# SuperScientificSoftwareLaboratory/PanguLU

Hardware: AMD Instinct MI355X
Metric: numeric factorisation GFLOP/s (pangulu_gstrf, R64) (higher is better)
Workload: dtype f64

## Files before the change

pangulu_amd/csrc/platform/pg_hip_front.h:

```cpp
#pragma once

#define FR_TILE 128
#define FR_KS 16
#define FR_LDA 144
#define FR_STAGE_DOUBLES (FR_KS * FR_LDA + FR_TILE * FR_KS)
#define FR_THREADS 512

typedef const char __attribute__((address_space(1))) *fr_gptr;
typedef void __attribute__((address_space(3))) *fr_lptr;

#ifndef FR_ISSUE_FIRST
#define FR_ISSUE_FIRST 0
#endif
#define FR_ORDER (FR_ISSUE_FIRST ? 0 : 1)
#ifndef FR_PRELOAD
#define FR_PRELOAD 1
#endif

template <int STAGES, bool PREFETCH, int ORDER>
__device__ __forceinline__ void fr_front_item(double *lds, const SsssmTaskD *__restrict__ tasks, int nb, const SsssmWorkD &G,
                                              unsigned long long *__restrict__ product_counter)
{
    const int tiles = nb / FR_TILE;
    const int tile = (int)G.tile;
    const int tid = threadIdx.x, lane = tid & 63;
    const int wave = __builtin_amdgcn_readfirstlane(tid >> 6);
    const int M0 = (tile % tiles) * FR_TILE, N0 = (tile / tiles) * FR_TILE;
    const int wm = (wave & 1) * 64, wn = (wave >> 1) * 32;
    const int l15 = lane & 15, l4 = lane >> 4;
    const int ntask = (int)(G.task_end - G.task_begin);
    const int steps_shift = nb == 256 ? 4 : 3;
    const int steps_per_task = 1 << steps_shift;
    const int T = ntask << steps_shift;
    const SsssmTaskD *my_tasks = tasks + G.task_begin;

    const unsigned a_voff = (unsigned)lane * 16u;
    const int bc = lane >> 3, bj = lane & 7;
    unsigned b_voff[2];
#pragma unroll
    for (int par = 0; par < 2; par++)
        b_voff[par] = ((unsigned)bc * (unsigned)nb + 2u * (unsigned)(bj ^ ((4 * par + (bc >> 1)) & 7))) * 8u;

    auto issue = [&](int st, fr_gptr pa, fr_gptr pb)
    {
        const int k0 = (st & (steps_per_task - 1)) * FR_KS;
        double *stage = lds + (st % STAGES) * FR_STAGE_DOUBLES;
#pragma unroll
        for (int h = 0; h < 2; h++)
        {
            const int k = wave + 8 * h;
            const fr_gptr src = dg_scalar_base(pa + ((size_t)(k0 + k) * nb + M0) * 8) + a_voff;
            __builtin_amdgcn_global_load_lds((const void __attribute__((address_space(1))) *)src, (fr_lptr)(stage + k * FR_LDA), 16, 0, 0);
        }
#pragma unroll
        for (int h = 0; h < 2; h++)
        {
            const int g = wave + 8 * h;
            const fr_gptr src = dg_scalar_base(pb + ((size_t)(N0 + 8 * g) * nb + k0) * 8) + b_voff[wave & 1];
            __builtin_amdgcn_global_load_lds((const void __attribute__((address_space(1))) *)src, (fr_lptr)(stage + FR_KS * FR_LDA + g * 128), 16, 0, 0);
        }
    };

    double __attribute__((address_space(1))) *C = (double __attribute__((address_space(1))) *)reinterpret_cast<double *>(G.cdense);
    const unsigned c_voff = ((unsigned)l4 * (unsigned)nb + (unsigned)l15) * 8u;
#define FR_C(ni_, mi_, r_)                                                                           \
    (*(double __attribute__((address_space(1))) *)(dg_scalar_base((const char __attribute__((address_space(1))) *)C +                    \
                                                                  ((size_t)(N0 + wn + (ni_) * 16 + 4 * (r_)) * nb + M0 + wm) * 8) + \
                                                   dg_lane_offset(c_voff) + (mi_) * 128))
    const bool preload = FR_PRELOAD && !G.atomic && T > 0;
    v4f64 acc[2][4];
#pragma unroll
    for (int ni = 0; ni < 2; ni++)
#pragma unroll
        for (int mi = 0; mi < 4; mi++)
        {
            if (preload)
            {
#pragma unroll
                for (int r = 0; r < 4; r++)
                    acc[ni][mi][r] = FR_C(ni, mi, r);
            }
            else
                acc[ni][mi] = (v4f64){0.0, 0.0, 0.0, 0.0};
        }

    fr_gptr pa_rq = nullptr, pb_rq = nullptr;
    if (T > 0)
    {
        pa_rq = (fr_gptr)reinterpret_cast<const char *>(my_tasks[0].a.val);
        pb_rq = (fr_gptr)reinterpret_cast<const char *>(my_tasks[0].b.val);
    }
#if PG_PLANES > 1
    bool add = T > 0 && my_tasks[0].sign < 0;
#endif

#pragma unroll
    for (int p = 0; p < STAGES - 1; p++)
        if (p < T)
            issue(p, pa_rq, pb_rq);

    const int a_frag = l4 * FR_LDA + wm + l15;
    int b_frag[2][2];
#pragma unroll
    for (int ni = 0; ni < 2; ni++)
    {
        const int n = wn + ni * 16 + l15;
        b_frag[ni][0] = FR_KS * FR_LDA + n * 16 + (l4 & 1);
        b_frag[ni][1] = (n >> 1) & 7;
    }

    for (int st = 0; st < T; st++)
    {
        const int rq = st + STAGES - 1;
        fr_gptr pa_nx = pa_rq, pb_nx = pb_rq;
        if (((rq + 1) & (steps_per_task - 1)) == 0 && rq + 1 < T)
        {
            const SsssmTaskD &Tn = my_tasks[(rq + 1) >> steps_shift];
            pa_nx = (fr_gptr)reinterpret_cast<const char *>(Tn.a.val);
            pb_nx = (fr_gptr)reinterpret_cast<const char *>(Tn.b.val);
        }
#if PG_PLANES > 1
        bool add_nx = add;
        if (((st + 1) & (steps_per_task - 1)) == 0 && st + 1 < T)
            add_nx = my_tasks[(st + 1) >> steps_shift].sign < 0;
#endif
        const int ahead = min(STAGES - 2, T - 1 - st);
        if (STAGES >= 4 && ahead >= 2)
            asm volatile("s_waitcnt vmcnt(8)" ::: "memory");
        else if (STAGES >= 3 && ahead >= 1)
            asm volatile("s_waitcnt vmcnt(4)" ::: "memory");
        else
            asm volatile("s_waitcnt vmcnt(0)" ::: "memory");
        __builtin_amdgcn_s_barrier();
        const bool request = rq < T;
        if (ORDER == 0 && request)
            issue(rq, pa_rq, pb_rq);
        const double *sA = lds + (st % STAGES) * FR_STAGE_DOUBLES;
#if PG_PLANES > 1
#define FR_MFMA(ni_, mi_, fb_, fa_)                                                                                        \
    if (add)                                                                                                                \
        acc[ni_][mi_] = __builtin_amdgcn_mfma_f64_16x16x4f64(fb_, fa_, acc[ni_][mi_], 0, 0, 0);                          \
    else                                                                                                                    \
        acc[ni_][mi_] = __builtin_amdgcn_mfma_f64_16x16x4f64(fb_, fa_, acc[ni_][mi_], 0, 0, DG_NEG_A);
#else
#define FR_MFMA(ni_, mi_, fb_, fa_) acc[ni_][mi_] = __builtin_amdgcn_mfma_f64_16x16x4f64(fb_, fa_, acc[ni_][mi_], 0, 0, DG_NEG_A);
#endif
#define FR_READ(fa_, fb_, kq_)                                                                        \
    {                                                                                                 \
        _Pragma("unroll") for (int mi = 0; mi < 4; mi++)(fa_)[mi] = sA[a_frag + (kq_) * 4 * FR_LDA + mi * 16]; \
        _Pragma("unroll") for (int ni = 0; ni < 2; ni++)(fb_)[ni] = sA[b_frag[ni][0] + 2 * ((2 * (kq_) + (l4 >> 1)) ^ b_frag[ni][1])]; \
    }
#define FR_REQUEST_BEHIND(kq_)                   \
    if (ORDER == 1 && (kq_) == 0 && request)     \
        issue(rq, pa_rq, pb_rq);
        if (PREFETCH)
        {
            double fa[2][4], fb[2][2];
            FR_READ(fa[0], fb[0], 0)
#pragma unroll
            for (int kq = 0; kq < FR_KS / 4; kq++)
            {
                if (kq + 1 < FR_KS / 4)
                    FR_READ(fa[(kq + 1) & 1], fb[(kq + 1) & 1], kq + 1)
#pragma unroll
                for (int ni = 0; ni < 2; ni++)
#pragma unroll
                    for (int mi = 0; mi < 4; mi++)
                    {
                        FR_MFMA(ni, mi, fb[kq & 1][ni], fa[kq & 1][mi])
                    }
                FR_REQUEST_BEHIND(kq)
            }
        }
        else
        {
#pragma unroll
            for (int kq = 0; kq < FR_KS / 4; kq++)
            {
                double fa[4], fb[2];
                FR_READ(fa, fb, kq)
#pragma unroll
                for (int ni = 0; ni < 2; ni++)
#pragma unroll
                    for (int mi = 0; mi < 4; mi++)
                    {
                        FR_MFMA(ni, mi, fb[ni], fa[mi])
                    }
                FR_REQUEST_BEHIND(kq)
            }
        }
#undef FR_REQUEST_BEHIND
#undef FR_READ
#undef FR_MFMA
        pa_rq = pa_nx;
        pb_rq = pb_nx;
#if PG_PLANES > 1
        add = add_nx;
#endif
    }
    if (product_counter && lane == 0 && T)
        atomicAdd(product_counter, (unsigned long long)(8 * T));

    if (preload)
    {
#pragma unroll
        for (int ni = 0; ni < 2; ni++)
#pragma unroll
            for (int mi = 0; mi < 4; mi++)
#pragma unroll
                for (int r = 0; r < 4; r++)
                    FR_C(ni, mi, r) = acc[ni][mi][r];
        return;
    }
#pragma unroll
    for (int ni = 0; ni < 2; ni++)
    {
        if (G.atomic)
        {
#pragma unroll
            for (int mi = 0; mi < 4; mi++)
#pragma unroll
                for (int r = 0; r < 4; r++)
                    atomicAdd((double *)&FR_C(ni, mi, r), acc[ni][mi][r]);
            continue;
        }
        double old[4][4];
#pragma unroll
        for (int mi = 0; mi < 4; mi++)
#pragma unroll
            for (int r = 0; r < 4; r++)
                old[mi][r] = FR_C(ni, mi, r);
#pragma unroll
        for (int mi = 0; mi < 4; mi++)
#pragma unroll
            for (int r = 0; r < 4; r++)
                FR_C(ni, mi, r) = old[mi][r] + acc[ni][mi][r];
    }
#undef FR_C
}

template <int STAGES, bool PREFETCH>
__global__ __launch_bounds__(FR_THREADS, (STAGES <= 2 ? 4 : 2)) void ssssm_front_f64_kernel(const SsssmTaskD *__restrict__ tasks, int nb, const SsssmWorkD *__restrict__ work,
                                                                     unsigned long long *__restrict__ product_counter, unsigned unit)
{
    __shared__ __align__(16) double lds[STAGES * FR_STAGE_DOUBLES];
    const int tiles = nb / FR_TILE;
    const unsigned bid = logical_block_id(unit ? unit : (unsigned)(tiles * tiles));
    const SsssmWorkD G = work[bid];
    fr_front_item<STAGES, PREFETCH, FR_ORDER>(lds, tasks, nb, G, product_counter);
}

#define TL_WINDOW 16
#ifndef TL_MARK
#define TL_PROBE_DECL
#define TL_MARK(i)
#define TL_PROBE_STEP
#define TL_PROBE_FLUSH
#endif
#ifndef TL_ITEM
#define TL_ITEM_DECL
#define TL_ITEM(i)
#define TL_ITEM_COUNT
#endif
#define TV_STEPS (TL_WINDOW * 16)
__global__ __launch_bounds__(FR_THREADS, 4) void ssssm_tilesv_f64_kernel(const SsssmTaskD *__restrict__ tasks, int nb, const SsssmWorkD *__restrict__ work,
                                                                          unsigned long long *__restrict__ product_counter, unsigned unit)
{
    __shared__ __align__(16) double lds[2 * FR_STAGE_DOUBLES];
    __shared__ unsigned long long s_spa[TV_STEPS], s_spb[TV_STEPS];
    __shared__ u32 s_step[TV_STEPS];
    __shared__ u32 s_cnt[FR_THREADS / 64];
#if PG_PLANES > 1
    __shared__ double s_sign[TL_WINDOW];
#endif
    const int tiles = nb / FR_TILE;
    const unsigned bid = logical_block_id(unit ? unit : (unsigned)(tiles * tiles));
    const SsssmWorkD G = work[bid];
    const int tile = (int)G.tile;
    const int tid = threadIdx.x, lane = tid & 63;
    const int wave = __builtin_amdgcn_readfirstlane(tid >> 6);
    const int M0 = (tile % tiles) * FR_TILE, N0 = (tile / tiles) * FR_TILE;
    const int wr = wave & 1, wc = wave >> 1;
    const int l15 = lane & 15, l4 = lane >> 4;
    if (G.pad_ != 0)
    {
        fr_front_item<2, true, FR_ORDER>(lds, tasks, nb, G, product_counter);
        return;
    }
    const int ntask = (int)(G.task_end - G.task_begin);
    const int nslab = nb / FR_KS;
    const SsssmTaskD *my_tasks = tasks + G.task_begin;

    const unsigned a_voff = (unsigned)lane * 16u;
    const int a_piece = lane >> 3;
    const int bc = lane >> 3, bj = lane & 7;
    const unsigned b_voff = ((unsigned)bc * (unsigned)nb + 2u * (unsigned)(bj ^ ((4 * (wave & 1) + (bc >> 1)) & 7))) * 8u;

    v4f64 acc[2][4];
#pragma unroll
    for (int ni = 0; ni < 2; ni++)
#pragma unroll
        for (int mi = 0; mi < 4; mi++)
            acc[ni][mi] = (v4f64){0.0, 0.0, 0.0, 0.0};
    unsigned touched = 0, nprod = 0;

    const int a_frag = l4 * FR_LDA + wr * 16 + l15;
    int b_frag[2][2];
#pragma unroll
    for (int ni = 0; ni < 2; ni++)
    {
        const int n = (wc + 4 * ni) * 16 + l15;
        b_frag[ni][0] = FR_KS * FR_LDA + n * 16 + (l4 & 1);
        b_frag[ni][1] = (n >> 1) & 7;
    }

    auto uniform64 = [&](unsigned long long v) -> fr_gptr
    { return (fr_gptr)(((unsigned long long)(unsigned)__builtin_amdgcn_readfirstlane((int)(v >> 32)) << 32) | (unsigned)__builtin_amdgcn_readfirstlane((int)v)); };
    auto issue = [&](unsigned w, fr_gptr pa, fr_gptr pb, int stage_no)
    {
        const unsigned ab = w & 0xFFu, bb = (w >> 8) & 0xFFu;
        const int k0 = (int)((w >> 16) & 15u) * FR_KS;
        double *stage = lds + stage_no * FR_STAGE_DOUBLES;
        const bool a_live = (ab >> a_piece) & 1u;
#pragma unroll
        for (int h = 0; h < 2; h++)
        {
            const int k = wave + 8 * h;
            const unsigned off = a_live ? (unsigned)(((k0 + k) * nb + M0) * 8) + a_voff : 0u;
            __builtin_amdgcn_global_load_lds((const void __attribute__((address_space(1))) *)(dg_scalar_base(pa) + off), (fr_lptr)(stage + k * FR_LDA), 16, 0, 0);
        }
#pragma unroll
        for (int h = 0; h < 2; h++)
        {
            const int g = wave + 8 * h;
            if (!((bb >> (g >> 1)) & 1u))
                continue;
            const unsigned off = (unsigned)(((N0 + 8 * g) * nb + k0) * 8) + b_voff;
            __builtin_amdgcn_global_load_lds((const void __attribute__((address_space(1))) *)(dg_scalar_base(pb) + off), (fr_lptr)(stage + FR_KS * FR_LDA + g * 128), 16, 0, 0);
        }
    };

    double __attribute__((address_space(1))) *C = (double __attribute__((address_space(1))) *)reinterpret_cast<double *>(G.cdense);
    const unsigned c_voff = ((unsigned)l4 * (unsigned)nb + (unsigned)l15) * 8u;
#define TL_C(ni_, mi_, r_)                                                                           \
    (*(double __attribute__((address_space(1))) *)(dg_scalar_base((const char __attribute__((address_space(1))) *)C +                    \
                                                                  ((size_t)(N0 + (wc + 4 * (ni_)) * 16 + 4 * (r_)) * nb + M0 + wr * 16) * 8) + \
                                                   dg_lane_offset(c_voff) + (mi_) * 256))
    unsigned pre = 0;
    const bool may_preload = !G.atomic && ntask <= TL_WINDOW;

    int stage_head = 0;
    TL_ITEM_DECL
    TL_ITEM_COUNT
    for (int win0 = 0; win0 < ntask; win0 += TL_WINDOW)
    {
        __syncthreads();
        int T;
        {
            unsigned v = 0;
            unsigned long long pa_v = 0, pb_v = 0;
            const int t_ = tid >> 4, s_ = tid & 15;
            if (tid < TL_WINDOW * 16 && win0 + t_ < ntask && s_ < nslab)
            {
                const SsssmTaskD &Tm = my_tasks[win0 + t_];
                const double *pa_ = reinterpret_cast<const double *>(Tm.a.val), *pb_ = reinterpret_cast<const double *>(Tm.b.val);
                pa_v = (unsigned long long)pa_;
                pb_v = (unsigned long long)pb_;
                unsigned ab_, bb_ = 0;
                if (Tm.has_map)
                {
                    ab_ = ((unsigned)Tm.amap[s_] >> (M0 / 16)) & 0xFFu;
                    bb_ = ((unsigned)Tm.bmap_t[s_] >> (N0 / 16)) & 0xFFu;
                }
                else
                {
                    ab_ = ((unsigned)mirror_map(pa_, nb)[s_] >> (M0 / 16)) & 0xFFu;
                    const uint4 mb_ = *reinterpret_cast<const uint4 *>(mirror_map(pb_, nb) + N0 / 16);
                    const unsigned w_[4] = {mb_.x, mb_.y, mb_.z, mb_.w};
#pragma unroll
                    for (int c_ = 0; c_ < 8; c_++)
                        bb_ |= (((w_[c_ >> 1] >> (16 * (c_ & 1))) >> s_) & 1u) << c_;
                }
                if (ab_ && bb_ && (!G.slab_mask || ((G.slab_mask >> s_) & 1u)))
                    v = (bb_ << 8) | ab_ | ((unsigned)s_ << 16) | ((unsigned)t_ << 20);
#if PG_PLANES > 1
                if (s_ == 0)
                    s_sign[t_] = Tm.sign;
#endif
            }
            const unsigned long long bal = __ballot(v != 0);
            TL_ITEM(0)
            if (lane == 0)
                s_cnt[wave] = (u32)__builtin_popcountll(bal);
            __syncthreads();
            unsigned at = (unsigned)__builtin_popcountll(bal & ((1ull << lane) - 1ull)), all = 0;
#pragma unroll
            for (int w_i = 0; w_i < FR_THREADS / 64; w_i++)
            {
                const unsigned c_ = s_cnt[w_i];
                at += w_i < wave ? c_ : 0u;
                all += c_;
            }
            if (v)
            {
                s_step[at] = v;
                s_spa[at] = pa_v;
                s_spb[at] = pb_v;
            }
            __syncthreads();
            T = __builtin_amdgcn_readfirstlane((int)all);
            TL_ITEM(1)
        }
        if (T == 0)
            continue;

        if (may_preload)
        {
            unsigned m = 0;
            for (int e = lane; e < T; e += 64)
            {
                const unsigned w = s_step[e];
                const unsigned ab = w & 0xFFu, bb = (w >> 8) & 0xFFu;
                const unsigned a4 = ((ab >> wr) & 1u) | (((ab >> (2 + wr)) & 1u) << 1) | (((ab >> (4 + wr)) & 1u) << 2) | (((ab >> (6 + wr)) & 1u) << 3);
                if ((bb >> wc) & 1u)
                    m |= a4;
                if ((bb >> (wc + 4)) & 1u)
                    m |= a4 << 4;
            }
#pragma unroll
            for (int off = 32; off > 0; off >>= 1)
                m |= (unsigned)__shfl_xor((int)m, off, 64);
            pre = (unsigned)__builtin_amdgcn_readfirstlane((int)m);
#pragma unroll
            for (int ni = 0; ni < 2; ni++)
#pragma unroll
                for (int mi = 0; mi < 4; mi++)
                    if ((pre >> (4 * ni + mi)) & 1u)
                    {
#pragma unroll
                        for (int r = 0; r < 4; r++)
                            acc[ni][mi][r] = TL_C(ni, mi, r);
                    }
        }
        TL_ITEM(2)
        unsigned wC = (unsigned)__builtin_amdgcn_readfirstlane((int)s_step[0]), wN = 0;
        fr_gptr paN = uniform64(s_spa[0]), pbN = uniform64(s_spb[0]);
        issue(wC, paN, pbN, stage_head);
        TL_ITEM(3)
        if (T > 1)
        {
            wN = (unsigned)__builtin_amdgcn_readfirstlane((int)s_step[1]);
            paN = uniform64(s_spa[1]);
            pbN = uniform64(s_spb[1]);
        }
        TL_PROBE_DECL
        for (int st = 0; st < T; st++)
        {
            TL_MARK(6)
            TL_PROBE_STEP
            const int e2 = min(st + 2, T - 1);
            const unsigned v_w = s_step[e2];
            const unsigned long long v_pa = s_spa[e2], v_pb = s_spb[e2];
            asm volatile("s_waitcnt vmcnt(0)" ::: "memory");
            TL_MARK(0)
            __builtin_amdgcn_s_barrier();
            TL_MARK(1)
            const unsigned w2 = (unsigned)__builtin_amdgcn_readfirstlane((int)v_w);
            const fr_gptr pa2 = uniform64(v_pa), pb2 = uniform64(v_pb);
            const double *sA = lds + ((stage_head + st) & 1) * FR_STAGE_DOUBLES;
            const unsigned ab = wC & 0xFFu, bb = (wC >> 8) & 0xFFu;
            const unsigned a4 = ((ab >> wr) & 1u) | (((ab >> (2 + wr)) & 1u) << 1) | (((ab >> (4 + wr)) & 1u) << 2) | (((ab >> (6 + wr)) & 1u) << 3);
            const unsigned b2 = ((bb >> wc) & 1u) | (((bb >> (wc + 4)) & 1u) << 1);
            const bool live = a4 && b2;
#if PG_PLANES > 1
            const bool add = s_sign[wC >> 20] < 0;
#endif
#define TV_READ(buf_, kq_)                                                                            \
    {                                                                                                 \
        _Pragma("unroll") for (int mi = 0; mi < 4; mi++) fa[buf_][mi] = sA[a_frag + (kq_) * 4 * FR_LDA + mi * 32]; \
        _Pragma("unroll") for (int ni = 0; ni < 2; ni++) fb[buf_][ni] = sA[b_frag[ni][0] + 2 * ((2 * (kq_) + (l4 >> 1)) ^ b_frag[ni][1])]; \
    }
            double fa[2][4], fb[2][2];
#define TV_PIECE2(ni_, mi_)                                                                                                            \
    if ((m8 >> ((mi_) + 4 * (ni_))) & 1u)                                                                                              \
    {                                                                                                                                   \
        TV_ONE(0, ni_, mi_)                                                                                                             \
        TV_ONE(1, ni_, mi_)                                                                                                             \
    }
#if PG_PLANES > 1
#define TV_ONE(buf_, ni_, mi_)                                                                                                          \
    if (add)                                                                                                                            \
        acc[ni_][mi_] = __builtin_amdgcn_mfma_f64_16x16x4f64(fb[buf_][ni_], fa[buf_][mi_], acc[ni_][mi_], 0, 0, 0);                     \
    else                                                                                                                                \
        acc[ni_][mi_] = __builtin_amdgcn_mfma_f64_16x16x4f64(fb[buf_][ni_], fa[buf_][mi_], acc[ni_][mi_], 0, 0, DG_NEG_A);
#else
#define TV_ONE(buf_, ni_, mi_) acc[ni_][mi_] = __builtin_amdgcn_mfma_f64_16x16x4f64(fb[buf_][ni_], fa[buf_][mi_], acc[ni_][mi_], 0, 0, DG_NEG_A);
#endif
#define TV_PAIR                                                                            \
    {                                                                                      \
        TV_PIECE2(0, 0) TV_PIECE2(0, 1) TV_PIECE2(0, 2) TV_PIECE2(0, 3)                    \
        TV_PIECE2(1, 0) TV_PIECE2(1, 1) TV_PIECE2(1, 2) TV_PIECE2(1, 3)                    \
    }
            unsigned m8 = 0;
            if (live)
            {
                m8 = ((b2 & 1u) ? a4 : 0u) | ((b2 & 2u) ? (a4 << 4) : 0u);
                nprod += (unsigned)__builtin_popcount(m8);
                touched |= m8;
                TV_READ(0, 0)
                TV_READ(1, 1)
                TV_PAIR
            }
            TL_MARK(2)
            if (st + 1 < T)
                issue(wN, paN, pbN, (stage_head + st + 1) & 1);
            TL_MARK(3)
            if (live)
            {
                TV_READ(0, 2)
                TV_READ(1, 3)
                TV_PAIR
            }
#undef TV_PIECE2
#undef TV_ONE
#undef TV_PAIR
#undef TV_READ
            wC = wN;
            wN = w2;
            paN = pa2;
            pbN = pb2;
            TL_MARK(4)
        }
        TL_PROBE_FLUSH
        stage_head = (stage_head + T) & 1;
        TL_ITEM(4)
    }
    if (product_counter && lane == 0 && nprod)
        atomicAdd(product_counter, (unsigned long long)nprod);

    if (pre)
    {
#pragma unroll
        for (int ni = 0; ni < 2; ni++)
#pragma unroll
            for (int mi = 0; mi < 4; mi++)
                if ((pre >> (4 * ni + mi)) & 1u)
                {
#pragma unroll
                    for (int r = 0; r < 4; r++)
                        TL_C(ni, mi, r) = acc[ni][mi][r];
                }
        touched = 0;
    }
#pragma unroll
    for (int ni = 0; ni < 2; ni++)
    {
        const unsigned t4 = (touched >> (4 * ni)) & 0xFu;
        if (!t4)
            continue;
        if (G.atomic)
        {
#pragma unroll
            for (int mi = 0; mi < 4; mi++)
            {
                if (!((t4 >> mi) & 1u))
                    continue;
#pragma unroll
                for (int r = 0; r < 4; r++)
                    if (acc[ni][mi][r] != 0.0)
                        atomicAdd((double *)&TL_C(ni, mi, r), acc[ni][mi][r]);
            }
            continue;
        }
        double old[4][4];
#pragma unroll
        for (int mi = 0; mi < 4; mi++)
#pragma unroll
            for (int r = 0; r < 4; r++)
                old[mi][r] = ((t4 >> mi) & 1u) ? TL_C(ni, mi, r) : 0.0;
#pragma unroll
        for (int mi = 0; mi < 4; mi++)
        {
            if (!((t4 >> mi) & 1u))
                continue;
#pragma unroll
            for (int r = 0; r < 4; r++)
                TL_C(ni, mi, r) = old[mi][r] + acc[ni][mi][r];
        }
    }
#ifdef TL_PROBE
    asm volatile("s_waitcnt vmcnt(0)" ::: "memory");
    TL_ITEM(5)
#endif
#undef TL_C
}
```

Measured before the change: 48850.

## Hand-schedule LDS reads and DMA issue in tiled SSSSM kernel inner loop

Rewrites the tilesv kernel's per-step loop to use inline-asm ds_read_b64 with precomputed per-kq LDS addresses and staggered lgkmcnt waits, so MFMAs start as soon as their operands arrive. Global-to-LDS copies now go through inline asm: the A rows are masked by setting EXEC with s_bitreplicate instead of redirecting dead lanes to offset 0, and fully-live steps get a fast path. The sign flag is packed into the step word in place of a shared-memory array, and sign handling negates the B fragment rather than branching between two MFMA variants. This aims to cut LDS latency stalls, branch overhead and wasted loads, at the cost of fragile hand-written waitcnt and exec management.

New measurement: 49460 (median of 6 runs). +1.2%, better.

```diff
diff --git a/pangulu_amd/csrc/platform/pg_hip_front.h b/pangulu_amd/csrc/platform/pg_hip_front.h
--- a/pangulu_amd/csrc/platform/pg_hip_front.h
+++ b/pangulu_amd/csrc/platform/pg_hip_front.h
@@ -136,19 +136,21 @@
         if (ORDER == 0 && request)
             issue(rq, pa_rq, pb_rq);
         const double *sA = lds + (st % STAGES) * FR_STAGE_DOUBLES;
+#define FR_MFMA(ni_, mi_, fb_, fa_) acc[ni_][mi_] = __builtin_amdgcn_mfma_f64_16x16x4f64(fb_, fa_, acc[ni_][mi_], 0, 0, DG_NEG_A);
 #if PG_PLANES > 1
-#define FR_MFMA(ni_, mi_, fb_, fa_)                                                                                        \
-    if (add)                                                                                                                \
-        acc[ni_][mi_] = __builtin_amdgcn_mfma_f64_16x16x4f64(fb_, fa_, acc[ni_][mi_], 0, 0, 0);                          \
-    else                                                                                                                    \
-        acc[ni_][mi_] = __builtin_amdgcn_mfma_f64_16x16x4f64(fb_, fa_, acc[ni_][mi_], 0, 0, DG_NEG_A);
+#define FR_FLIP(fb_)                                               \
+    if (add)                                                       \
+    {                                                              \
+        _Pragma("unroll") for (int ni = 0; ni < 2; ni++)(fb_)[ni] = -(fb_)[ni]; \
+    }
 #else
-#define FR_MFMA(ni_, mi_, fb_, fa_) acc[ni_][mi_] = __builtin_amdgcn_mfma_f64_16x16x4f64(fb_, fa_, acc[ni_][mi_], 0, 0, DG_NEG_A);
+#define FR_FLIP(fb_)
 #endif
 #define FR_READ(fa_, fb_, kq_)                                                                        \
     {                                                                                                 \
         _Pragma("unroll") for (int mi = 0; mi < 4; mi++)(fa_)[mi] = sA[a_frag + (kq_) * 4 * FR_LDA + mi * 16]; \
         _Pragma("unroll") for (int ni = 0; ni < 2; ni++)(fb_)[ni] = sA[b_frag[ni][0] + 2 * ((2 * (kq_) + (l4 >> 1)) ^ b_frag[ni][1])]; \
+        FR_FLIP(fb_)                                                                                  \
     }
 #define FR_REQUEST_BEHIND(kq_)                   \
     if (ORDER == 1 && (kq_) == 0 && request)     \
@@ -191,6 +193,7 @@
         }
 #undef FR_REQUEST_BEHIND
 #undef FR_READ
+#undef FR_FLIP
 #undef FR_MFMA
         pa_rq = pa_nx;
         pb_rq = pb_nx;
@@ -270,9 +273,6 @@
     __shared__ unsigned long long s_spa[TV_STEPS], s_spb[TV_STEPS];
     __shared__ u32 s_step[TV_STEPS];
     __shared__ u32 s_cnt[FR_THREADS / 64];
-#if PG_PLANES > 1
-    __shared__ double s_sign[TL_WINDOW];
-#endif
     const int tiles = nb / FR_TILE;
     const unsigned bid = logical_block_id(unit ? unit : (unsigned)(tiles * tiles));
     const SsssmWorkD G = work[bid];
@@ -292,7 +292,6 @@
     const SsssmTaskD *my_tasks = tasks + G.task_begin;
 
     const unsigned a_voff = (unsigned)lane * 16u;
-    const int a_piece = lane >> 3;
     const int bc = lane >> 3, bj = lane & 7;
     const unsigned b_voff = ((unsigned)bc * (unsigned)nb + 2u * (unsigned)(bj ^ ((4 * (wave & 1) + (bc >> 1)) & 7))) * 8u;
 
@@ -304,39 +303,79 @@
             acc[ni][mi] = (v4f64){0.0, 0.0, 0.0, 0.0};
     unsigned touched = 0, nprod = 0;
 
-    const int a_frag = l4 * FR_LDA + wr * 16 + l15;
-    int b_frag[2][2];
-#pragma unroll
-    for (int ni = 0; ni < 2; ni++)
-    {
-        const int n = (wc + 4 * ni) * 16 + l15;
-        b_frag[ni][0] = FR_KS * FR_LDA + n * 16 + (l4 & 1);
-        b_frag[ni][1] = (n >> 1) & 7;
-    }
+    const unsigned lds0 = (unsigned)(__UINTPTR_TYPE__)(fr_lptr)lds;
+    unsigned a_addr = lds0 + (unsigned)(l4 * FR_LDA + wr * 16 + l15) * 8u;
+    unsigned b_addr[4];
+#pragma unroll
+    for (int kq = 0; kq < 4; kq++)
+        b_addr[kq] = lds0 + (unsigned)(FR_KS * FR_LDA + (wc * 16 + l15) * 16 + (l4 & 1) + 2 * ((2 * kq + (l4 >> 1)) ^ ((l15 >> 1) & 7))) * 8u;
+#define TV_STAGE_BYTES (FR_STAGE_DOUBLES * 8)
+#define TV_DSR(dst_, addr_, off_) asm volatile("ds_read_b64 %0, %1 offset:%2" : "=v"(dst_) : "v"(addr_), "n"(off_) : "memory");
+#define TV_READS(kqa_, kqb_)                                                                           \
+    TV_DSR(fb[0][0], b_addr[kqa_], 0)                                              \
+    TV_DSR(fa[0][0], a_addr, (kqa_) * 4 * FR_LDA * 8)                          \
+    TV_DSR(fb[1][0], b_addr[kqb_], 0)                                              \
+    TV_DSR(fa[1][0], a_addr, (kqb_) * 4 * FR_LDA * 8)                          \
+    TV_DSR(fa[0][1], a_addr, (kqa_) * 4 * FR_LDA * 8 + 256)                    \
+    TV_DSR(fa[1][1], a_addr, (kqb_) * 4 * FR_LDA * 8 + 256)                    \
+    TV_DSR(fa[0][2], a_addr, (kqa_) * 4 * FR_LDA * 8 + 512)                    \
+    TV_DSR(fa[1][2], a_addr, (kqb_) * 4 * FR_LDA * 8 + 512)                    \
+    TV_DSR(fa[0][3], a_addr, (kqa_) * 4 * FR_LDA * 8 + 768)                    \
+    TV_DSR(fa[1][3], a_addr, (kqb_) * 4 * FR_LDA * 8 + 768)                    \
+    TV_DSR(fb[0][1], b_addr[kqa_], 8192)                                       \
+    TV_DSR(fb[1][1], b_addr[kqb_], 8192)
+#define TV_WAIT2(n_, x0_, x1_) asm volatile("s_waitcnt lgkmcnt(" #n_ ")" : "+v"(x0_), "+v"(x1_)::"memory");
+#define TV_WAIT4(n_, x0_, x1_, x2_, x3_) asm volatile("s_waitcnt lgkmcnt(" #n_ ")" : "+v"(x0_), "+v"(x1_), "+v"(x2_), "+v"(x3_)::"memory");
 
     auto uniform64 = [&](unsigned long long v) -> fr_gptr
     { return (fr_gptr)(((unsigned long long)(unsigned)__builtin_amdgcn_readfirstlane((int)(v >> 32)) << 32) | (unsigned)__builtin_amdgcn_readfirstlane((int)v)); };
+#define TV_DMA(voff_, base_, m0_) \
+    asm volatile("s_mov_b32 m0, %2\n\ts_nop 0\n\tglobal_load_lds_dwordx4 %0, %1" ::"v"(voff_), "s"(base_), "s"(m0_) : "memory");
+#define TV_DMA_LANES(voff_, base_, m0_, mask_)                                                                                        \
+    {                                                                                                                                  \
+        unsigned long long exec_;                                                                                                      \
+        asm volatile("s_mov_b64 %0, exec\n\ts_mov_b64 exec, %4\n\ts_mov_b32 m0, %3\n\ts_nop 0\n\tglobal_load_lds_dwordx4 %1, %2\n\ts_mov_b64 exec, %0" \
+                     : "=&s"(exec_)                                                                                                    \
+                     : "v"(voff_), "s"(base_), "s"(m0_), "s"(mask_)                                                                    \
+                     : "memory");                                                                                                      \
+    }
     auto issue = [&](unsigned w, fr_gptr pa, fr_gptr pb, int stage_no)
     {
         const unsigned ab = w & 0xFFu, bb = (w >> 8) & 0xFFu;
         const int k0 = (int)((w >> 16) & 15u) * FR_KS;
-        double *stage = lds + stage_no * FR_STAGE_DOUBLES;
-        const bool a_live = (ab >> a_piece) & 1u;
+        const unsigned stage = lds0 + (unsigned)stage_no * (unsigned)TV_STAGE_BYTES;
+        unsigned long long a_base[2], b_base[2];
+        unsigned a_m0[2], b_m0[2];
 #pragma unroll
         for (int h = 0; h < 2; h++)
         {
-            const int k = wave + 8 * h;
-            const unsigned off = a_live ? (unsigned)(((k0 + k) * nb + M0) * 8) + a_voff : 0u;
-            __builtin_amdgcn_global_load_lds((const void __attribute__((address_space(1))) *)(dg_scalar_base(pa) + off), (fr_lptr)(stage + k * FR_LDA), 16, 0, 0);
-        }
+            const int k = wave + 8 * h, g = wave + 8 * h;
+            a_base[h] = (unsigned long long)pa + (unsigned)(((k0 + k) * nb + M0) * 8);
+            a_m0[h] = stage + (unsigned)(k * FR_LDA * 8);
+            b_base[h] = (unsigned long long)pb + (unsigned)(((N0 + 8 * g) * nb + k0) * 8);
+            b_m0[h] = stage + (unsigned)((FR_KS * FR_LDA + g * 128) * 8);
+        }
+        if ((w & 0xFFFFu) == 0xFFFFu)
+        {
+            TV_DMA(a_voff, a_base[0], a_m0[0])
+            TV_DMA(a_voff, a_base[1], a_m0[1])
+            TV_DMA(b_voff, b_base[0], b_m0[0])
+            TV_DMA(b_voff, b_base[1], b_m0[1])
+            return;
+        }
+        unsigned long long a_lanes;
+        asm("s_bitreplicate_b64_b32 %0, %1" : "=s"(a_lanes) : "s"(ab));
+        asm("s_bitreplicate_b64_b32 %0, %1" : "=s"(a_lanes) : "s"((unsigned)a_lanes));
+        asm("s_bitreplicate_b64_b32 %0, %1" : "=s"(a_lanes) : "s"((unsigned)a_lanes));
+        TV_DMA_LANES(a_voff, a_base[0], a_m0[0], a_lanes)
+        TV_DMA_LANES(a_voff, a_base[1], a_m0[1], a_lanes)
 #pragma unroll
         for (int h = 0; h < 2; h++)
         {
             const int g = wave + 8 * h;
             if (!((bb >> (g >> 1)) & 1u))
                 continue;
-            const unsigned off = (unsigned)(((N0 + 8 * g) * nb + k0) * 8) + b_voff;
-            __builtin_amdgcn_global_load_lds((const void __attribute__((address_space(1))) *)(dg_scalar_base(pb) + off), (fr_lptr)(stage + FR_KS * FR_LDA + g * 128), 16, 0, 0);
+            TV_DMA(b_voff, b_base[h], b_m0[h])
         }
     };
 
@@ -349,7 +388,7 @@
     unsigned pre = 0;
     const bool may_preload = !G.atomic && ntask <= TL_WINDOW;
 
-    int stage_head = 0;
+    int stage_cur = 0;
     TL_ITEM_DECL
     TL_ITEM_COUNT
     for (int win0 = 0; win0 < ntask; win0 += TL_WINDOW)
@@ -382,11 +421,12 @@
                         bb_ |= (((w_[c_ >> 1] >> (16 * (c_ & 1))) >> s_) & 1u) << c_;
                 }
                 if (ab_ && bb_ && (!G.slab_mask || ((G.slab_mask >> s_) & 1u)))
+                {
                     v = (bb_ << 8) | ab_ | ((unsigned)s_ << 16) | ((unsigned)t_ << 20);
 #if PG_PLANES > 1
-                if (s_ == 0)
-                    s_sign[t_] = Tm.sign;
-#endif
+                    v |= Tm.sign < 0 ? 1u << 24 : 0u;
+#endif
+                }
             }
             const unsigned long long bal = __ballot(v != 0);
             TL_ITEM(0)
@@ -445,7 +485,7 @@
         TL_ITEM(2)
         unsigned wC = (unsigned)__builtin_amdgcn_readfirstlane((int)s_step[0]), wN = 0;
         fr_gptr paN = uniform64(s_spa[0]), pbN = uniform64(s_spb[0]);
-        issue(wC, paN, pbN, stage_head);
+        issue(wC, paN, pbN, stage_cur);
         TL_ITEM(3)
         if (T > 1)
         {
@@ -454,33 +494,13 @@
             pbN = uniform64(s_spb[1]);
         }
         TL_PROBE_DECL
-        for (int st = 0; st < T; st++)
-        {
-            TL_MARK(6)
-            TL_PROBE_STEP
-            const int e2 = min(st + 2, T - 1);
-            const unsigned v_w = s_step[e2];
-            const unsigned long long v_pa = s_spa[e2], v_pb = s_spb[e2];
-            asm volatile("s_waitcnt vmcnt(0)" ::: "memory");
-            TL_MARK(0)
-            __builtin_amdgcn_s_barrier();
-            TL_MARK(1)
-            const unsigned w2 = (unsigned)__builtin_amdgcn_readfirstlane((int)v_w);
-            const fr_gptr pa2 = uniform64(v_pa), pb2 = uniform64(v_pb);
-            const double *sA = lds + ((stage_head + st) & 1) * FR_STAGE_DOUBLES;
-            const unsigned ab = wC & 0xFFu, bb = (wC >> 8) & 0xFFu;
-            const unsigned a4 = ((ab >> wr) & 1u) | (((ab >> (2 + wr)) & 1u) << 1) | (((ab >> (4 + wr)) & 1u) << 2) | (((ab >> (6 + wr)) & 1u) << 3);
-            const unsigned b2 = ((bb >> wc) & 1u) | (((bb >> (wc + 4)) & 1u) << 1);
-            const bool live = a4 && b2;
-#if PG_PLANES > 1
-            const bool add = s_sign[wC >> 20] < 0;
-#endif
-#define TV_READ(buf_, kq_)                                                                            \
-    {                                                                                                 \
-        _Pragma("unroll") for (int mi = 0; mi < 4; mi++) fa[buf_][mi] = sA[a_frag + (kq_) * 4 * FR_LDA + mi * 32]; \
-        _Pragma("unroll") for (int ni = 0; ni < 2; ni++) fb[buf_][ni] = sA[b_frag[ni][0] + 2 * ((2 * (kq_) + (l4 >> 1)) ^ b_frag[ni][1])]; \
-    }
-            double fa[2][4], fb[2][2];
+#define TV_WAIT_SLAB                  \
+    __builtin_amdgcn_s_waitcnt(0x0F70); \
+    asm volatile("" ::: "memory");
+#define TV_RECORD                                                                                     \
+    asm volatile("" : "+v"(v_w), "+v"(v_pa), "+v"(v_pb));                                             \
+    const unsigned w2 = (unsigned)__builtin_amdgcn_readfirstlane((int)v_w);                           \
+    const fr_gptr pa2 = uniform64(v_pa), pb2 = uniform64(v_pb);
 #define TV_PIECE2(ni_, mi_)                                                                                                            \
     if ((m8 >> ((mi_) + 4 * (ni_))) & 1u)                                                                                              \
     {                                                                                                                                   \
@@ -488,51 +508,100 @@
         TV_ONE(1, ni_, mi_)                                                                                                             \
     }
 #if PG_PLANES > 1
-#define TV_ONE(buf_, ni_, mi_)                                                                                                          \
-    if (add)                                                                                                                            \
-        acc[ni_][mi_] = __builtin_amdgcn_mfma_f64_16x16x4f64(fb[buf_][ni_], fa[buf_][mi_], acc[ni_][mi_], 0, 0, 0);                     \
-    else                                                                                                                                \
-        acc[ni_][mi_] = __builtin_amdgcn_mfma_f64_16x16x4f64(fb[buf_][ni_], fa[buf_][mi_], acc[ni_][mi_], 0, 0, DG_NEG_A);
+#define TV_FLIP(x_) \
+    if (add)        \
+        x_ = -x_;
 #else
+#define TV_FLIP(x_)
+#endif
 #define TV_ONE(buf_, ni_, mi_) acc[ni_][mi_] = __builtin_amdgcn_mfma_f64_16x16x4f64(fb[buf_][ni_], fa[buf_][mi_], acc[ni_][mi_], 0, 0, DG_NEG_A);
-#endif
 #define TV_PAIR                                                                            \
     {                                                                                      \
-        TV_PIECE2(0, 0) TV_PIECE2(0, 1) TV_PIECE2(0, 2) TV_PIECE2(0, 3)                    \
+        TV_WAIT4(8, fb[0][0], fa[0][0], fb[1][0], fa[1][0])                                \
+        TV_FLIP(fb[0][0]) TV_FLIP(fb[1][0])                                                \
+        TV_PIECE2(0, 0)                                                                    \
+        TV_WAIT2(6, fa[0][1], fa[1][1])                                                    \
+        TV_PIECE2(0, 1)                                                                    \
+        TV_WAIT2(4, fa[0][2], fa[1][2])                                                    \
+        TV_PIECE2(0, 2)                                                                    \
+        TV_WAIT2(2, fa[0][3], fa[1][3])                                                    \
+        TV_PIECE2(0, 3)                                                                    \
+        TV_WAIT2(0, fb[0][1], fb[1][1])                                                    \
+        TV_FLIP(fb[0][1]) TV_FLIP(fb[1][1])                                                \
         TV_PIECE2(1, 0) TV_PIECE2(1, 1) TV_PIECE2(1, 2) TV_PIECE2(1, 3)                    \
     }
-            unsigned m8 = 0;
-            if (live)
-            {
-                m8 = ((b2 & 1u) ? a4 : 0u) | ((b2 & 2u) ? (a4 << 4) : 0u);
-                nprod += (unsigned)__builtin_popcount(m8);
-                touched |= m8;
-                TV_READ(0, 0)
-                TV_READ(1, 1)
-                TV_PAIR
-            }
-            TL_MARK(2)
-            if (st + 1 < T)
-                issue(wN, paN, pbN, (stage_head + st + 1) & 1);
-            TL_MARK(3)
-            if (live)
-            {
-                TV_READ(0, 2)
-                TV_READ(1, 3)
-                TV_PAIR
-            }
+#define TV_STEP                                                                                                                         \
+    {                                                                                                                                   \
+        TL_MARK(6)                                                                                                                      \
+        TL_PROBE_STEP                                                                                                                   \
+        const int e2 = min(st + 2, T - 1);                                                                                              \
+        unsigned v_w = s_step[e2];                                                                                                      \
+        unsigned long long v_pa = s_spa[e2], v_pb = s_spb[e2];                                                                          \
+        TV_WAIT_SLAB                                                                                                                    \
+        TL_MARK(0)                                                                                                                      \
+        __builtin_amdgcn_s_barrier();                                                                                                   \
+        TL_MARK(1)                                                                                                                      \
+        double fa[2][4], fb[2][2];                                                                                                      \
+        unsigned w2_;                                                                                                                   \
+        fr_gptr pa2_, pb2_;                                                                                                             \
+        {                                                                                                                               \
+            const unsigned ab = wC & 0xFFu, bb = (wC >> 8) & 0xFFu;                                                                     \
+            const unsigned a4 = ((ab >> wr) & 1u) | (((ab >> (2 + wr)) & 1u) << 1) | (((ab >> (4 + wr)) & 1u) << 2) | (((ab >> (6 + wr)) & 1u) << 3); \
+            const unsigned b2 = ((bb >> wc) & 1u) | (((bb >> (wc + 4)) & 1u) << 1);                                                     \
+            const bool live = a4 && b2;                                                                                                 \
+            TV_ADD_DECL                                                                                                                 \
+            unsigned m8 = 0;                                               \
+            if (live)                                                                                                                   \
+            {                                                                                                                           \
+                m8 = ((b2 & 1u) ? a4 : 0u) | ((b2 & 2u) ? (a4 << 4) : 0u);                                                              \
+                nprod += (unsigned)__builtin_popcount(m8);                                                                              \
+                touched |= m8;                                                                                                          \
+                TV_READS(0, 1)                                                                                                          \
+                TV_PAIR                                                                                                                 \
+            }                                                                                                                           \
+            TL_MARK(2)                                                                                                                  \
+            TV_RECORD                                                                                                                   \
+                                                                            \
+            if (st + 1 < T)                                                                                                             \
+                issue(wN, paN, pbN, stage_cur ^ 1);                                                                                          \
+            TL_MARK(3)                                                                                                                  \
+            if (m8)                                                                                                                     \
+            {                                                                                                                           \
+                TV_READS(2, 3)                                                                                                          \
+                TV_PAIR                                                                                                                 \
+            }                                                                                                                           \
+            w2_ = w2, pa2_ = pa2, pb2_ = pb2;                                                                                           \
+        }                                                                                                                               \
+        wC = wN;                                                                                                                        \
+        wN = w2_;                                                                                                                       \
+        paN = pa2_;                                                                                                                     \
+        pbN = pb2_;                                                                                                                     \
+        TL_MARK(4)                                                                                                                      \
+    }
+#if PG_PLANES > 1
+#define TV_ADD_DECL const bool add = (wC >> 24) & 1u;
+#else
+#define TV_ADD_DECL
+#endif
+        for (int st = 0; st < T; st++)
+        {
+            TV_STEP
+            const unsigned hop = stage_cur ? 0u - (unsigned)TV_STAGE_BYTES : (unsigned)TV_STAGE_BYTES;
+            a_addr += hop;
+#pragma unroll
+            for (int kq = 0; kq < 4; kq++)
+                b_addr[kq] += hop;
+            stage_cur ^= 1;
+        }
+#undef TV_STEP
+#undef TV_ADD_DECL
+#undef TV_RECORD
+#undef TV_WAIT_SLAB
 #undef TV_PIECE2
 #undef TV_ONE
+#undef TV_FLIP
 #undef TV_PAIR
-#undef TV_READ
-            wC = wN;
-            wN = w2;
-            paN = pa2;
-            pbN = pb2;
-            TL_MARK(4)
-        }
         TL_PROBE_FLUSH
-        stage_head = (stage_head + T) & 1;
         TL_ITEM(4)
     }
     if (product_counter && lane == 0 && nprod)
@@ -593,4 +662,11 @@
     TL_ITEM(5)
 #endif
 #undef TL_C
+#undef TV_DMA_LANES
+#undef TV_DMA
+#undef TV_WAIT4
+#undef TV_WAIT2
+#undef TV_READS
+#undef TV_DSR
+#undef TV_STAGE_BYTES
 }
```
